# gui-yupeng/sesr-pytorch-quantize

Measured on AMD Instinct MI355X. Metric: INT8 SESR frames/sec (whole job) + PSNR-vs-ref-sim (bit-exact), higher is better.
Workload: dtype i8

## Files before the change

sesr-pytorch-quantize_amd/csrc/sesrq_trio.hip:

```cpp
#include <stdlib.h>

#include <algorithm>
#include <mutex>
#include <type_traits>

#include "sesrq_mfma_common.h"

namespace sesrq {

#ifdef SESRQ_STAMPS
__device__ unsigned long long g_trio_stamps[1024 * 4 * 12 * 8];
#define TSTAMP(k)                                                                                                         \
    if (l == 0 && stamp_step < 12) {                                                                                      \
        const unsigned wg_ = (blockIdx.z * gridDim.y + blockIdx.y) * gridDim.x + blockIdx.x;                              \
        if (wg_ < 1024) g_trio_stamps[((wg_ * 4 + w) * 12 + stamp_step) * 8 + (k)] = __builtin_amdgcn_s_memtime();          \
    }
#else
#define TSTAMP(k)
#endif

constexpr int TV = 60;
constexpr int TH = 8;
constexpr int TP = 66;
constexpr int TR = TH + 2;
constexpr int OOB = (int)0x80000000;
constexpr int TRIO_WIN = TR * TP + 2;
constexpr int TRIO_LUT_I4 = 32;
constexpr int TRIO_LDS_BYTES = 3 * TRIO_WIN * 16;

struct TrioStage {
    static constexpr int NIT = 3;
    v4u v[NIT];
    bool ok[NIT];
    int voff[NIT], ty[NIT], tx[NIT];
    int voff2s;
    __amdgpu_buffer_rsrc_t rs;
    int row_bytes;
    __device__ __forceinline__ void init(const TrioArgs &a, int n_img, int x0, int tid) {
        const size_t img = (size_t)a.H * a.W * 16;
        rs = __builtin_amdgcn_make_buffer_rsrc((char *)const_cast<void *>(a.in) + (size_t)n_img * img, 0, (int)img, 0x00020000);
        row_bytes = a.W * 16;
#pragma unroll
        for (int it = 0; it < NIT; ++it) {
            const int i = tid + it * 256;
            ty[it] = i / TP;
            tx[it] = i - ty[it] * TP;
            const int gx = x0 - 1 + tx[it];
            const bool okx = (gx >= 0) & (gx < a.W) & (i < TR * TP);
            voff[it] = okx ? (ty[it] * a.W + gx) * 16 : OOB;
            if (!okx) ty[it] = NO_ROW;
        }
        voff2s = (ty[2] < TH) ? voff[2] : OOB;
    }
    template <bool COLD>
    __device__ __forceinline__ void load(const TrioArgs &a, int y) {
        constexpr int nrows = COLD ? TR : TH;
        const int lo = -y, hi = min(a.H - y, nrows);
#pragma unroll
        for (int it = 0; it < NIT; ++it) {
            ok[it] = (ty[it] >= lo) & (ty[it] < hi);
            if constexpr (COLD) v[it] = __builtin_amdgcn_raw_buffer_load_b128(rs, ok[it] ? voff[it] + y * row_bytes : OOB, 0, 0);
            else v[it] = __builtin_amdgcn_raw_buffer_load_b128(rs, it == 2 ? voff2s : voff[it], y * row_bytes, 0);
        }
    }
    template <bool COLD>
    __device__ __forceinline__ void store(int4 *win, int pad_word, int tid) const {
        constexpr int nrows = COLD ? TR : TH, pos0 = COLD ? 0 : 2;
        const unsigned pw = (unsigned)pad_word;
#pragma unroll
        for (int it = 0; it < NIT; ++it) {
            const int i = tid + it * 256;
            const v4u pad = {pw, pw, pw, pw};
            const v4u t = ok[it] ? v[it] : pad;
            if (i < nrows * TP) win[pos0 * TP + i] = make_int4((int)t[0], (int)t[1], (int)t[2], (int)t[3]);
        }
    }
};

struct TrioEpiC {
    float Mf, sh, z_next, Mres, shres, z_merge, Md, Cd;
};

struct TrioArgsQ : TrioArgs {
    float qlo, qhi, qhalf, qspan;
};
#define SESRQ_KERNEL mfma_trio_kernel
#define SESRQ_NARROW 0
#define SESRQ_TRIO_ARGS TrioArgs
#define SESRQ_TRIO_TEMPLATE template <int EPI_C, int U8>
#include "sesrq_trio_kernel.inc"
#undef SESRQ_KERNEL
#undef SESRQ_NARROW
#undef SESRQ_TRIO_ARGS
#undef SESRQ_TRIO_TEMPLATE
#define SESRQ_KERNEL mfma_trio_kernel_q
#define SESRQ_NARROW 1
#define SESRQ_TRIO_ARGS TrioArgsQ
#define SESRQ_TRIO_TEMPLATE template <int EPI_C, int U8 = 0>
#include "sesrq_trio_kernel.inc"
#undef SESRQ_KERNEL
#undef SESRQ_NARROW
#undef SESRQ_TRIO_ARGS
#undef SESRQ_TRIO_TEMPLATE

template <auto KERN, int REG = REG_MAIN, class ARGS = TrioArgs>
static void launch_trio_k(ARGS a, hipStream_t st) {
    constexpr int occ = 4;
    const int lds = std::max(TRIO_LDS_BYTES, ((160 * 1024 / occ) & ~1023) - TRIO_LUT_I4 * 16);
    const int strips = (a.W + TV - 1) / TV, steps = (a.H + TH - 1) / TH;
    const RunCut c = cut_runs(strips, steps, a.N, a.wg_budget, occ * device_cu_count());
    a.chunk_steps = c.chunk; a.inv_nx = c.inv_nx;
    a.run_unit = (steps < 3 * c.k) ? TH / 2 : TH;
    const int units = (a.H + a.run_unit - 1) / a.run_unit;
    a.run_q = units / c.k; a.run_rem = units % c.k;
    dim3 grid(strips, c.k, a.N);
    launch_kernel<KERN, REG>(grid, dim3(256), (unsigned)lds, st, a);
}

#ifdef SESRQ_STAMPS
extern "C" int sesrq_debug_fetch_trio_stamps(void *host, size_t bytes) {
    return (int)hipMemcpyFromSymbol(host, HIP_SYMBOL(g_trio_stamps), std::min(bytes, sizeof(g_trio_stamps)), 0, hipMemcpyDeviceToHost);
}
#endif

constexpr bool trio_built(int epi, int u8) {
    return (epi == EPI_MID || epi == EPI_PRERES) && (u8 == 0 || u8 == 1 || u8 == 3 || u8 == 7 || (u8 == 15 && epi == EPI_PRERES));
}
static int select_trio(const TrioArgs &a, int epi_c) {
    bool u8 = a.l[0].z_next == -128.f && a.l[1].z_next == -128.f && a.l[0].zlo == -128.f && a.l[1].zlo == -128.f;
    if (epi_c == EPI_PRERES) u8 = u8 && a.z_merge == -128.f;
    else u8 = u8 && a.l[2].z_next == -128.f && a.l[2].zlo == -128.f;
    u8 = u8 && (a.allow & 1);
    const bool ab = u8 && (a.allow & 2) && a.l[0].direct && a.l[1].direct, abc = ab && (a.allow & 4) && a.l[2].direct;
    if (abc && epi_c == EPI_PRERES && a.rc_in == a.in && (a.allow & 8)) return 15;
    return abc ? 7 : (ab ? 3 : (u8 ? 1 : 0));
}

int launch_trio(const TrioArgs &a, int epi_c, hipStream_t st) {
    if (!frame_fits_32bit_offsets(a.H, a.W)) { set_error("trio: frame too large for 32-bit buffer offsets (H*W must stay below 2^24 pixels)"); return 1; }
    const bool built = pick([&](auto E, auto U) {
        if constexpr (trio_built(E, U)) return launch_trio_k<mfma_trio_kernel<E, U>>(a, st), true; else return false;
    }, Of<EPI_MID, EPI_PRERES>{}, epi_c, Of<0, 1, 3, 7, 15>{}, select_trio(a, epi_c));
    if (!built) { set_error("trio: the third layer must be a hidden layer"); return 1; }
    return check_launch("trio");
}

int launch_trio_q(const TrioArgs &a, const ConvArgs &width, int epi_c, hipStream_t st) {
    if (!frame_fits_32bit_offsets(a.H, a.W)) { set_error("trio: frame too large for 32-bit buffer offsets (H*W must stay below 2^24 pixels)"); return 1; }
    TrioArgsQ q;
    static_cast<TrioArgs &>(q) = a;
    q.qlo = width.qlo; q.qhi = width.qhi; q.qhalf = width.qhalf; q.qspan = width.qspan;
    const bool built = pick([&](auto E) { return launch_trio_k<mfma_trio_kernel_q<E>, REG_NARROW, TrioArgsQ>(q, st), true; }, Of<EPI_MID, EPI_PRERES>{}, epi_c);
    if (!built) { set_error("trio: the third layer must be a hidden layer"); return 1; }
    return check_launch("trio");
}

}
```

sesr-pytorch-quantize_amd/csrc/sesrq_trio_kernel.inc:

```
SESRQ_TRIO_TEMPLATE
__global__ __launch_bounds__(256) void SESRQ_KERNEL(const SESRQ_TRIO_ARGS a) {
    constexpr bool NARROW = SESRQ_NARROW != 0;
    using ARGS = SESRQ_TRIO_ARGS;
    extern __shared__ int4 trio_lds[];
    __shared__ int4 trio_lut[TRIO_LUT_I4];
    int4 *lutp = trio_lut, *bufI = trio_lds, *bufA = bufI + TRIO_WIN, *bufB = bufI + 2 * TRIO_WIN;
    QRange qr = {};
    if constexpr (NARROW) qr = qrange(a);
    constexpr bool LUT = EPI_C == EPI_PRERES;
    constexpr bool RCW = LUT && (U8 & 8) != 0;
    const float lut_magic = MAGIC + 256.f + (float)(unsigned)(size_t)(const __attribute__((address_space(3))) void *)lutp;
    const int tid = threadIdx.x, w = tid >> 6, l = tid & 63, n = l & 15, g = l >> 4;
    kernarg_warm<ARGS>();
    const BlockXY bxy = xcd_block(a.inv_nx);
    const int n_img = blockIdx.z;
    const int x0 = bxy.x * TV - 2;
    const int u_begin = bxy.y * a.run_q + min(bxy.y, a.run_rem);
    const int y_begin = a.run_unit * u_begin;
    const int y_end = a.run_unit * (u_begin + a.run_q + (bxy.y < a.run_rem ? 1 : 0));
    if (y_begin >= y_end) return;
    TrioStage st;
    st.init(a, n_img, x0, tid);
    st.load<true>(a, y_begin - TH + 1);
    int lut_word = 0;
    if constexpr (LUT) {
        if (threadIdx.x < 128) lut_word = a.merge_lut[threadIdx.x];
    }

    const int c = 16 * w + n, gx = x0 + c;
    const bool col_in = (gx >= 0) & (gx < a.W);
    const bool col_out = (c >= 2) & (c < 2 + TV) & (gx < a.W);
    const bool strip_in = (x0 >= 0) & (x0 + 63 < a.W);
    const int rdcol = c + g;
    const int wrcol = (c + 1) * 4 + g;

    v4i A[3][3], acc0[3];
#pragma unroll
    for (int k = 0; k < 3; ++k) {
        const int4 ac = a.l[k].afrag[g];
        acc0[k] = (v4i){ac.x + MAGIC_I, ac.y + MAGIC_I, ac.z + MAGIC_I, ac.w + MAGIC_I};
#pragma unroll
        for (int f = 0; f < 3; ++f) A[k][f] = ld_frag(a.l[k].afrag + 4 + f * 64 + l);
    }
    const size_t img = (size_t)a.H * a.W * 16;
    RowIO io;
    io.out = __builtin_amdgcn_make_buffer_rsrc((char *)a.out + (size_t)n_img * img, 0, (int)img, 0x00020000);
    io.rc_in = __builtin_amdgcn_make_buffer_rsrc((char *)const_cast<void *>(a.rc_in) + (size_t)n_img * img, 0, (int)img, 0x00020000);
    io.rc_out = io.out;
    io.row_bytes = a.W * 16;
    const int voff_c = col_out ? (g * a.W + gx) * 16 : OOB;
    const TrioEpiC ec = {a.l[2].Mf, a.l[2].sh, a.l[2].z_next, a.Mres, a.shres, a.z_merge, a.l[2].Md, a.l[2].Cd};

    auto inner = [&](auto KC, auto I0, auto I1, const int4 *src, int4 *dst, int row0, auto PADC) __attribute__((always_inline)) {
        constexpr int K = decltype(KC)::value, i0 = decltype(I0)::value, i1 = decltype(I1)::value;
        constexpr bool PAD = decltype(PADC)::value;
        const TrioLayer &L = a.l[K];
        const int4 *p = src + rdcol;
        unsigned *d = reinterpret_cast<unsigned *>(dst) + wrcol;
        v4i B0 = ld_frag(p + (i0)*TP), B1 = ld_frag(p + (i0 + 1) * TP);
#pragma unroll
        for (int i = i0; i < i1; ++i) {
            const v4i B2 = ld_frag(p + (i + 2) * TP);
            v4i acc = mfma(A[K][0], B0, acc0[K]);
            acc = mfma(A[K][1], B1, acc);
            acc = mfma(A[K][2], B2, acc);
            B0 = B1; B1 = B2;
            const int s[4] = {acc[0], acc[1], acc[2], acc[3]};
            unsigned q;
            if constexpr (NARROW) q = epi_mid_q<true>(s, L, L.zlo, qr);
            else q = epi_mid<true, (U8 & 2) ? 2 : (U8 & 1)>(s, L, L.zlo);
            if constexpr (PAD) {
                const int row = row0 + i;
                const bool rok = (row >= 0) & (row < a.H);
                q = (rok & col_in) ? q : (unsigned)L.pad_next;
            }
            d[(2 + i) * TP * 4] = q;
        }
    };
    auto rc_fetch = [&](auto NRC, int Y, v4u (&rcp)[2]) __attribute__((always_inline)) {
        constexpr int NR = decltype(NRC)::value;
        if constexpr (LUT) {
            const int vo = col_out ? voff_c + Y * io.row_bytes : OOB;
#pragma unroll
            for (int y4 = 0; y4 < NR; y4 += 4) rcp[y4 / 4] = __builtin_amdgcn_raw_buffer_load_b128(io.rc_in, vo, y4 * io.row_bytes, 0);
        }
    };
    auto outer = [&](auto NRC, int Y, const v4u (&rcp)[2]) __attribute__((always_inline)) {
        constexpr int NR = decltype(NRC)::value;
        const int4 *p = bufB + rdcol;
        io.voff = col_out ? voff_c + Y * io.row_bytes : OOB;
        v4i B0 = ld_frag(p), B1 = ld_frag(p + TP);
#pragma unroll
        for (int y4 = 0; y4 < NR; y4 += 4) {
            int s4[4][4];
#pragma unroll
            for (int r = 0; r < 4; ++r) {
                const v4i B2 = ld_frag(p + (y4 + r + 2) * TP);
                v4i acc = mfma(A[2][0], B0, acc0[2]);
                acc = mfma(A[2][1], B1, acc);
                acc = mfma(A[2][2], B2, acc);
                B0 = B1; B1 = B2;
#pragma unroll
                for (int i = 0; i < 4; ++i) s4[r][i] = acc[i];
            }
            if constexpr (LUT) {
                const v4u rv = rcp[y4 / 4];
                unsigned rcw[4] = {rv[0], rv[1], rv[2], rv[3]}, wq[4];
                if constexpr (!RCW) transpose4(rcw);
#pragma unroll
                for (int r = 0; r < 4; ++r) {
                    if constexpr (NARROW) wq[r] = epi_preres_lut_q<true>(s4[r], rcw[r], ec, lut_magic, qr);
                    else wq[r] = epi_preres_lut<true, (U8 & 4) != 0>(s4[r], rcw[r], ec, lut_magic,
                                                                    (const unsigned char __attribute__((address_space(3))) *)lutp);
                }
                store_rows4(io.out, io, y4, wq);
            } else if constexpr (NARROW) {
                emit_rows4_q<EPI_C, false, true>(s4, ec, io, y4, a.l[2].zlo, qr);
            } else {
                emit_rows4<EPI_C, false, true, (U8 & 4) ? 2 : (U8 & 1)>(s4, ec, io, y4, a.l[2].zlo);
            }
        }
    };
    auto rc_win = [&](int pos) __attribute__((always_inline)) { return (unsigned)reinterpret_cast<const int *>(bufI)[pos * TP * 4 + wrcol]; };
    unsigned rcc = 0;
    auto rc_from_window = [&](auto NRC, v4u (&rcp)[2]) __attribute__((always_inline)) {
        constexpr int NR = decltype(NRC)::value;
        unsigned t[8] = {0, 0, 0, 0, 0, 0, 0, 0};
#pragma unroll
        for (int i = 0; i < NR; ++i) t[i] = rc_win(i);
        rcp[0] = (v4u){rcc, t[0], t[1], t[2]};
        if constexpr (NR == 8) { rcp[1] = (v4u){t[3], t[4], t[5], t[6]}; rcc = t[7]; }
    };
    using std::integral_constant;
    auto shift = [&](int4 *win) __attribute__((always_inline)) {
        if (tid < 2 * TP) { const int4 t = win[TH * TP + tid]; win[tid] = t; }
    };

    using IC0 = integral_constant<int, 0>;
    using IC1 = integral_constant<int, 1>;
    using IC4 = integral_constant<int, 4>;
    using IC6 = integral_constant<int, 6>;
    using IC8 = integral_constant<int, 8>;
    {
        const int Y = y_begin - TH;
        st.store<true>(bufI, a.pad_in, tid);
        if constexpr (LUT) {
            if (threadIdx.x < 128) reinterpret_cast<int *>(lutp)[threadIdx.x] = lut_word;
        }
        __syncthreads();
        if constexpr (RCW) rcc = rc_win(TH - 1);
        st.load<false>(a, Y + TH + 3);
        inner(IC0(), IC4(), IC8(), bufI, bufA, Y + 2, std::true_type());
        int4 shI = make_int4(0, 0, 0, 0);
        if (tid < 2 * TP) shI = bufI[TH * TP + tid];
        __syncthreads();
        if (tid < 2 * TP) bufI[tid] = shI;
        st.store<false>(bufI, a.pad_in, tid);
        inner(IC1(), IC6(), IC8(), bufA, bufB, Y + 1, std::true_type());
        __syncthreads();
        shift(bufA);
        __syncthreads();
    }
    int Y = y_begin;
#ifdef SESRQ_STAMPS
    int stamp_step = 0;
#endif
    int4 shB = make_int4(0, 0, 0, 0);
    if (tid < 2 * TP) shB = bufB[TH * TP + tid];
    for (; y_end - Y >= TH; Y += TH) {
        TSTAMP(0)
        const bool more = Y + TH < y_end;
        if (more) st.load<false>(a, Y + TH + 3);
        v4u rcp[2] = {{0, 0, 0, 0}, {0, 0, 0, 0}};
        if constexpr (RCW) rc_from_window(IC8(), rcp);
        const bool nopad = strip_in && (Y + TH + 2 <= a.H);
        if (nopad) inner(IC0(), IC0(), IC8(), bufI, bufA, Y + 2, std::false_type());
        else inner(IC0(), IC0(), IC8(), bufI, bufA, Y + 2, std::true_type());
        int4 shI = make_int4(0, 0, 0, 0);
        if (tid < 2 * TP) shI = bufI[TH * TP + tid];
        TSTAMP(1)
        __syncthreads();
        TSTAMP(2)
        if (tid < 2 * TP) bufB[tid] = shB;
        if (more && tid < 2 * TP) bufI[tid] = shI;
        if constexpr (!RCW) rc_fetch(IC8(), Y, rcp);
        TSTAMP(3)
        if (nopad) inner(IC1(), IC0(), IC8(), bufA, bufB, Y + 1, std::false_type());
        else inner(IC1(), IC0(), IC8(), bufA, bufB, Y + 1, std::true_type());
        if (more) st.store<false>(bufI, a.pad_in, tid);
        int4 shA = make_int4(0, 0, 0, 0);
        if (tid < 2 * TP) shA = bufA[TH * TP + tid];
        TSTAMP(4)
        __syncthreads();
        TSTAMP(5)
        if (tid < 2 * TP) bufA[tid] = shA;
        outer(IC8(), Y, rcp);
        if (tid < 2 * TP) shB = bufB[TH * TP + tid];
        TSTAMP(6)
        TSTAMP(7)
#ifdef SESRQ_STAMPS
        ++stamp_step;
#endif
    }
    if (Y < y_end) {
        v4u rcp[2] = {{0, 0, 0, 0}, {0, 0, 0, 0}};
        if constexpr (RCW) rc_from_window(IC4(), rcp);
        inner(IC0(), IC0(), IC4(), bufI, bufA, Y + 2, std::true_type());
        __syncthreads();
        if (tid < 2 * TP) bufB[tid] = shB;
        if constexpr (!RCW) rc_fetch(IC4(), Y, rcp);
        inner(IC1(), IC0(), IC4(), bufA, bufB, Y + 1, std::true_type());
        __syncthreads();
        outer(IC4(), Y, rcp);
    }
}
```

Before: 19170.

## Load trio input halo directly into LDS with buffer_load lds

Replaces register-staged global loads followed by LDS stores with inline-asm buffer_load_dwordx4 ... lds, which writes input rows straight into the shared window via M0. The loads are issued later, after the previous window rows are shifted, and a settle step waits on vmcnt and then fills out-of-bounds cells with the pad value only at frame edges. This removes the VGPRs holding staged tiles and the LDS write instructions, which may help occupancy. In exchange the load now overlaps less with the first inner stage, and the hand-written M0 and waitcnt asm carries correctness risk.

```diff
diff --git a/sesr-pytorch-quantize_amd/csrc/sesrq_trio.hip b/sesr-pytorch-quantize_amd/csrc/sesrq_trio.hip
--- a/sesr-pytorch-quantize_amd/csrc/sesrq_trio.hip
+++ b/sesr-pytorch-quantize_amd/csrc/sesrq_trio.hip
@@ -30,49 +30,57 @@
 
 struct TrioStage {
     static constexpr int NIT = 3;
-    v4u v[NIT];
-    bool ok[NIT];
-    int voff[NIT], ty[NIT], tx[NIT];
-    int voff2s;
-    __amdgpu_buffer_rsrc_t rs;
+    int voff[NIT], ty[NIT];
+    v4i rs;
     int row_bytes;
+    unsigned lds0;
+    bool cols_in;
     __device__ __forceinline__ void init(const TrioArgs &a, int n_img, int x0, int tid) {
         const size_t img = (size_t)a.H * a.W * 16;
-        rs = __builtin_amdgcn_make_buffer_rsrc((char *)const_cast<void *>(a.in) + (size_t)n_img * img, 0, (int)img, 0x00020000);
+        const unsigned long long base = (unsigned long long)a.in + (unsigned long long)n_img * img;
+        rs = (v4i){(int)(unsigned)base, (int)(unsigned)(base >> 32) & 0xffff, (int)img, 0x00020000};
         row_bytes = a.W * 16;
+        lds0 = (unsigned)__builtin_amdgcn_readfirstlane(tid >> 6) * 64 * 16;
+        cols_in = (x0 >= 1) & (x0 + TP - 2 < a.W);
 #pragma unroll
         for (int it = 0; it < NIT; ++it) {
             const int i = tid + it * 256;
             ty[it] = i / TP;
-            tx[it] = i - ty[it] * TP;
-            const int gx = x0 - 1 + tx[it];
+            const int tx = i - ty[it] * TP;
+            const int gx = x0 - 1 + tx;
             const bool okx = (gx >= 0) & (gx < a.W) & (i < TR * TP);
             voff[it] = okx ? (ty[it] * a.W + gx) * 16 : OOB;
             if (!okx) ty[it] = NO_ROW;
         }
-        voff2s = (ty[2] < TH) ? voff[2] : OOB;
+    }
+    static __device__ __forceinline__ void piece(const v4i &rs, int voffset, int soffset, unsigned lds) {
+        unsigned keep;
+        asm volatile("s_mov_b32 %0, m0\n\ts_mov_b32 m0, %3\n\ts_nop 0\n\tbuffer_load_dwordx4 %1, %2, %4 offen lds\n\ts_mov_b32 m0, %0"
+                     : "=&s"(keep) : "v"(voffset), "s"(rs), "s"(lds), "s"(soffset) : "memory");
     }
     template <bool COLD>
-    __device__ __forceinline__ void load(const TrioArgs &a, int y) {
-        constexpr int nrows = COLD ? TR : TH;
+    __device__ __forceinline__ void load(const TrioArgs &a, const int4 *win, int y, int tid) const {
+        constexpr int nrows = COLD ? TR : TH, pos0 = COLD ? 0 : 2;
+        const unsigned dst = (unsigned)(size_t)(const __attribute__((address_space(3))) void *)win + pos0 * TP * 16 + lds0;
         const int lo = -y, hi = min(a.H - y, nrows);
 #pragma unroll
         for (int it = 0; it < NIT; ++it) {
-            ok[it] = (ty[it] >= lo) & (ty[it] < hi);
-            if constexpr (COLD) v[it] = __builtin_amdgcn_raw_buffer_load_b128(rs, ok[it] ? voff[it] + y * row_bytes : OOB, 0, 0);
-            else v[it] = __builtin_amdgcn_raw_buffer_load_b128(rs, it == 2 ? voff2s : voff[it], y * row_bytes, 0);
+            int vo = voff[it], so = y * row_bytes;
+            if constexpr (COLD) { vo = ((ty[it] >= lo) & (ty[it] < hi)) ? vo + so : OOB; so = 0; }
+            if ((it + 1) * 256 <= nrows * TP || tid + it * 256 < nrows * TP) piece(rs, vo, so, dst + it * 256 * 16);
         }
     }
     template <bool COLD>
-    __device__ __forceinline__ void store(int4 *win, int pad_word, int tid) const {
+    __device__ __forceinline__ void settle(const TrioArgs &a, int4 *win, int y, int tid) const {
         constexpr int nrows = COLD ? TR : TH, pos0 = COLD ? 0 : 2;
-        const unsigned pw = (unsigned)pad_word;
+        asm volatile("s_waitcnt vmcnt(0)" ::: "memory");
+        if (cols_in & (y >= 0) & (y + nrows <= a.H)) return;
+        const int lo = -y, hi = min(a.H - y, nrows);
 #pragma unroll
         for (int it = 0; it < NIT; ++it) {
             const int i = tid + it * 256;
-            const v4u pad = {pw, pw, pw, pw};
-            const v4u t = ok[it] ? v[it] : pad;
-            if (i < nrows * TP) win[pos0 * TP + i] = make_int4((int)t[0], (int)t[1], (int)t[2], (int)t[3]);
+            const bool ok = (ty[it] >= lo) & (ty[it] < hi);
+            if (!ok && i < nrows * TP) win[pos0 * TP + i] = make_int4(a.pad_in, a.pad_in, a.pad_in, a.pad_in);
         }
     }
 };
diff --git a/sesr-pytorch-quantize_amd/csrc/sesrq_trio_kernel.inc b/sesr-pytorch-quantize_amd/csrc/sesrq_trio_kernel.inc
--- a/sesr-pytorch-quantize_amd/csrc/sesrq_trio_kernel.inc
+++ b/sesr-pytorch-quantize_amd/csrc/sesrq_trio_kernel.inc
@@ -21,7 +21,7 @@
     if (y_begin >= y_end) return;
     TrioStage st;
     st.init(a, n_img, x0, tid);
-    st.load<true>(a, y_begin - TH + 1);
+    st.load<true>(a, bufI, y_begin - TH + 1, tid);
     int lut_word = 0;
     if constexpr (LUT) {
         if (threadIdx.x < 128) lut_word = a.merge_lut[threadIdx.x];
@@ -143,20 +143,20 @@
     using IC8 = integral_constant<int, 8>;
     {
         const int Y = y_begin - TH;
-        st.store<true>(bufI, a.pad_in, tid);
+        st.settle<true>(a, bufI, Y + 1, tid);
         if constexpr (LUT) {
             if (threadIdx.x < 128) reinterpret_cast<int *>(lutp)[threadIdx.x] = lut_word;
         }
         __syncthreads();
         if constexpr (RCW) rcc = rc_win(TH - 1);
-        st.load<false>(a, Y + TH + 3);
         inner(IC0(), IC4(), IC8(), bufI, bufA, Y + 2, std::true_type());
         int4 shI = make_int4(0, 0, 0, 0);
         if (tid < 2 * TP) shI = bufI[TH * TP + tid];
         __syncthreads();
         if (tid < 2 * TP) bufI[tid] = shI;
-        st.store<false>(bufI, a.pad_in, tid);
+        st.load<false>(a, bufI, Y + TH + 3, tid);
         inner(IC1(), IC6(), IC8(), bufA, bufB, Y + 1, std::true_type());
+        st.settle<false>(a, bufI, Y + TH + 3, tid);
         __syncthreads();
         shift(bufA);
         __syncthreads();
@@ -170,7 +170,6 @@
     for (; y_end - Y >= TH; Y += TH) {
         TSTAMP(0)
         const bool more = Y + TH < y_end;
-        if (more) st.load<false>(a, Y + TH + 3);
         v4u rcp[2] = {{0, 0, 0, 0}, {0, 0, 0, 0}};
         if constexpr (RCW) rc_from_window(IC8(), rcp);
         const bool nopad = strip_in && (Y + TH + 2 <= a.H);
@@ -183,11 +182,12 @@
         TSTAMP(2)
         if (tid < 2 * TP) bufB[tid] = shB;
         if (more && tid < 2 * TP) bufI[tid] = shI;
+        if (more) st.load<false>(a, bufI, Y + TH + 3, tid);
         if constexpr (!RCW) rc_fetch(IC8(), Y, rcp);
         TSTAMP(3)
         if (nopad) inner(IC1(), IC0(), IC8(), bufA, bufB, Y + 1, std::false_type());
         else inner(IC1(), IC0(), IC8(), bufA, bufB, Y + 1, std::true_type());
-        if (more) st.store<false>(bufI, a.pad_in, tid);
+        if (more) st.settle<false>(a, bufI, Y + TH + 3, tid);
         int4 shA = make_int4(0, 0, 0, 0);
         if (tid < 2 * TP) shA = bufA[TH * TP + tid];
         TSTAMP(4)
```

Result: slower. 18500 (-3.5%).
